# Junshuai-Song/Graph-Embedding

Hardware: AMD Instinct MI355X
Metric: walk-steps/sec (node2vec) (higher is better)
Workload: dtype int32 ids / f64 accept tests

## Files before the change

graph-embedding_amd/csrc/gw_n2v_bitset.hip:

```cpp
#include <hip/hip_runtime.h>
#include <hipcub/hipcub.hpp>

#include <algorithm>
#include <cstdlib>
#include <string>
#include <vector>

#include "gw_device_common.h"

namespace {

constexpr int kB = 256;
constexpr int kBlk = 16;
constexpr int kDirBits = 512;
constexpr int kStage = 16;

constexpr int kPDir = 8;

__host__ __device__ __forceinline__ int64_t bs_ndir(int64_t d) { return d > kDirBits ? (d + kDirBits - 1) / kDirBits : 0; }
__host__ __device__ __forceinline__ int64_t bs_round(int64_t w) { return (w + kBlk - 1) / kBlk * kBlk; }
__host__ __device__ __forceinline__ int64_t bs_boff(int64_t d) {
  return (gw_bs_is_inline((uint32_t)d) || bs_ndir(d) <= kPDir) ? 0 : bs_round(bs_ndir(d));
}
__host__ __device__ __forceinline__ int64_t bs_words(int64_t d) {
  return gw_bs_is_inline((uint32_t)d) ? 0 : bs_boff(d) + bs_round((d + 31) / 32);
}

__device__ __forceinline__ bool bs_has_edge(const gw_dev_graph& G, int64_t rb, int64_t re, int32_t key) {
  if (G.eh) return gw_eh_has(G.eh, rb, re, key);
  if (G.bitmap) {
    const uint32_t h = (uint32_t)key * 0x9E3779B1u;
    const uint64_t bit = 16ull * (uint64_t)rb + (((uint64_t)h * (uint64_t)(16 * (re - rb))) >> 32);
    if (!((G.bitmap[bit >> 5] >> (bit & 31)) & 1u)) return false;
  }
  return gw_row_find(G.nbrs, rb, re, key) >= 0;
}

__host__ __device__ __forceinline__ uint32_t bs_filt_buckets(int64_t ndir, uint32_t d) {
  return 32u * (gw_bs_pw(d) - ((ndir > 0 && ndir <= kPDir) ? 5u : 1u));
}
__host__ __device__ __forceinline__ uint32_t bs_filt_word(int64_t ndir) { return (ndir > 0 && ndir <= kPDir) ? 5u : 1u; }

__device__ __forceinline__ int word_select(uint32_t x, uint32_t j) {
  int pos = 0;
#pragma unroll
  for (int w = 16; w >= 1; w >>= 1) {
    const uint32_t lowc = (uint32_t)__popc(x & ((1u << w) - 1u));
    if (j >= lowc) {
      j -= lowc;
      x >>= w;
      pos += w;
    }
  }
  return pos;
}


enum { BS_LIST = 0, BS_INLINE = 1, BS_EF = 2, BS_REGION = 3 };
constexpr uint32_t kFiltL = 320;

__device__ __forceinline__ int64_t bs_div32(int64_t k, uint32_t d, double inv, bool* exact) {
  int64_t q = (int64_t)((double)k * inv);
  int64_t r = (k << 32) - q * (int64_t)d;
  if (r < 0) {
    --q;
    r += d;
  } else if (r >= (int64_t)d) {
    ++q;
    r -= d;
  }
  *exact = r == 0;
  return q;
}
__device__ __forceinline__ void bs_draw_range(int64_t k, uint32_t d, double inv, uint32_t* ylo, uint32_t* yhi) {
  bool ex;
  *ylo = (uint32_t)bs_div32(k, d, inv, &ex);
  const int64_t q1 = bs_div32(k + 1, d, inv, &ex);
  *yhi = (uint32_t)(q1 - (ex ? 1 : 0));
}
__device__ __forceinline__ double bs_inv32(uint32_t d) { return 4294967296.0 / (double)d; }

__device__ __forceinline__ void bs_filter_only(uint32_t* w, int64_t k, uint32_t d, double inv) {
  uint32_t ulo, uhi;
  bs_draw_range(k, d, inv, &ulo, &uhi);
  const uint32_t b0 = gw_bounded(ulo, kFiltL), b1 = gw_bounded(uhi, kFiltL);
  for (uint32_t b = b0; b <= b1; ++b) atomicOr(&w[b >> 5], 1u << (b & 31));
}
__device__ __forceinline__ int bs_mode(uint32_t c, uint32_t d) {
  return gw_bs_is_list(c, d) ? BS_LIST : gw_bs_is_inline(d) ? BS_INLINE : gw_bs_is_ef(c, d) ? BS_EF : BS_REGION;
}

constexpr uint32_t kDualC = 6;
constexpr uint32_t kMetaDual = 0x40000000u;
constexpr uint32_t kMetaStash = 0x80000000u;

__device__ __forceinline__ uint32_t bs_meta(uint32_t c, uint32_t d) {
  const uint32_t mode = (uint32_t)bs_mode(c, d);
  uint32_t l = 0, U = 0;
  if (mode == BS_EF) {
    l = (uint32_t)gw_bs_ef_l(c, d);
    U = c + ((d - 1) >> l) + 1;
  }
  const uint32_t bblk = (mode == BS_REGION) ? (uint32_t)(bs_boff(d) / kBlk) : 0u;
  return mode | (l << 2) | (U << 7) | (bblk << 16);
}
__device__ __forceinline__ bool bs_dual(uint32_t c, uint32_t c_rev, uint32_t d, uint32_t du) {
  return c <= kDualC && c_rev <= kDualC && d < GW_BS_PACK_D && du < GW_BS_PACK_D;
}
__device__ __forceinline__ uint32_t bs_meta_slot(uint32_t c, uint32_t c_rev, uint32_t d, uint32_t du) {
  return bs_dual(c, c_rev, d, du) ? (kMetaDual | (c_rev << 2)) : bs_meta(c, d);
}

struct BsEmit {
  int mode;
  bool nobits;
  uint32_t* w;
  uint32_t* dir;
  uint16_t* pdir;
  uint32_t* bits;
  int64_t ndir;
  uint32_t d;
  double inv;
  int l;
  uint32_t U;
  __device__ void operator()(int64_t k, uint32_t idx, int64_t kprev) const {
    const uint32_t bit = 1u << (k & 31);
    if (mode == BS_LIST) {
      reinterpret_cast<uint16_t*>(w)[idx] = (uint16_t)k;
    } else if (mode == BS_INLINE) {
      atomicOr(&w[k >> 5], bit);
    } else if (mode == BS_EF) {
      const uint32_t hp = (uint32_t)(k >> l) + idx;
      atomicOr(&w[hp >> 5], 1u << (hp & 31));
      if (l > 0) {
        const uint32_t lowv = (uint32_t)k & ((1u << l) - 1u), off = U + idx * (uint32_t)l, sh = off & 31;
        atomicOr(&w[off >> 5], lowv << sh);
        if (sh + (uint32_t)l > 32u) atomicOr(&w[(off >> 5) + 1], lowv >> (32 - sh));
      }
    } else {
      if (!nobits) atomicOr(&bits[k >> 5], bit);
      set_dir((kprev < 0 ? -1 : kprev / kDirBits) + 1, k / kDirBits, idx);
      uint32_t ulo, uhi;
      bs_draw_range(k, d, inv, &ulo, &uhi);
      const uint32_t F = bs_filt_buckets(ndir, d), w0 = bs_filt_word(ndir);
      const uint32_t b0 = gw_bounded(ulo, F), b1 = gw_bounded(uhi, F);
      for (uint32_t b = b0; b <= b1; ++b) atomicOr(&w[w0 + (b >> 5)], 1u << (b & 31));
    }
  }
  __device__ void set_dir(int64_t g0, int64_t g1, uint32_t count) const {
    if (ndir == 0) return;
    for (int64_t g = g0; g <= g1 && g < ndir; ++g) {
      if (pdir)
        pdir[g] = (uint16_t)count;
      else
        dir[g] = count;
    }
  }
};

__device__ __forceinline__ uint32_t* bs_payload(gw_bs_nbr* en, uint32_t d) { return en->r + (d < GW_BS_PACK_D ? 1 : 2); }
__device__ __forceinline__ uint32_t bs_c(const gw_bs_nbr* en, uint32_t d) { return d < GW_BS_PACK_D ? en->r[0] >> 16 : en->r[1]; }

__device__ __forceinline__ BsEmit bs_emit(gw_bs_nbr* en, uint32_t* reg, const uint64_t* roff, int64_t e, uint32_t c,
                                          uint32_t d) {
  BsEmit E;
  E.mode = bs_mode(c, d);
  E.nobits = false;
  E.w = bs_payload(en, d);
  E.ndir = 0;
  E.dir = E.bits = nullptr;
  E.pdir = nullptr;
  E.d = d;
  E.inv = bs_inv32(d);
  E.l = 0;
  E.U = 0;
  if (E.mode == BS_EF) {
    E.l = gw_bs_ef_l(c, d);
    E.U = c + ((d - 1) >> E.l) + 1;
  } else if (E.mode == BS_REGION) {
    E.ndir = bs_ndir(d);
    E.dir = reg + roff[e];
    E.bits = E.dir + bs_boff(d);
    if (E.ndir <= kPDir) {
      E.pdir = reinterpret_cast<uint16_t*>(E.w + 1);
      E.dir = nullptr;
    }
  }
  return E;
}

__global__ void k_bs_sizes(gw_dev_graph G, const gw_bs_nbr* __restrict__ bsn, uint64_t* __restrict__ sz,
                           int lists_only) {
  const int64_t e = (int64_t)blockIdx.x * blockDim.x + threadIdx.x;
  if (e >= G.nnz) return;
  const uint32_t d = (uint32_t)G.deg[G.nbrs[e]];
  sz[e] = (!lists_only && !gw_bs_is_inline(d) && bs_mode(bs_c(bsn + e, d), d) == BS_REGION)
              ? (uint64_t)bs_words(d) : 0ull;
}

constexpr int kTB = 512;
constexpr int kTW = kTB / 64;
constexpr int kTriH = 4096;
constexpr int kTriS = 2 * kTriH;
constexpr int kTriEB = 512;
constexpr int kTriAhead = 4;
constexpr int32_t kTriNotOwned = INT32_MIN;

constexpr double kBuildProbeRate = 7.7e10;
constexpr double kBuildSlotSeconds = 5.0e-11;

struct TriItem {
  int32_t u, j0;
};

__global__ void k_bs_iota(int64_t n, int32_t* __restrict__ a) {
  const int64_t i = (int64_t)blockIdx.x * blockDim.x + threadIdx.x;
  if (i < n) a[i] = (int32_t)i;
}

__global__ void k_bs_nitems(gw_dev_graph G, const int32_t* __restrict__ order, uint32_t* __restrict__ nit) {
  const int64_t i = (int64_t)blockIdx.x * blockDim.x + threadIdx.x;
  if (i > G.n) return;
  nit[i] = i < G.n ? (uint32_t)((G.deg[order[i]] + kTriEB - 1) / kTriEB) : 0u;
}

__global__ void k_bs_items(gw_dev_graph G, const int32_t* __restrict__ order, const uint32_t* __restrict__ itoff,
                           TriItem* __restrict__ items) {
  const int64_t i = (int64_t)blockIdx.x * blockDim.x + threadIdx.x;
  if (i >= G.n) return;
  const int32_t u = order[i];
  const uint32_t b = itoff[i], e = itoff[i + 1];
  for (uint32_t t = b; t < e; ++t) items[t] = TriItem{u, (int32_t)((t - b) * kTriEB)};
}

struct TriSlot {
  BsEmit E;
  uint32_t* gw;
  bool filt;
  bool dual;
  __device__ void operator()(int64_t k, uint32_t idx, int64_t kprev) const {
    if (filt)
      bs_filter_only(E.w, k, E.d, E.inv);
    else
      E(k, idx, kprev);
  }
};

__device__ __forceinline__ TriSlot tri_slot(gw_bs_nbr* en, uint32_t* reg, const uint64_t* roff, int64_t e, uint32_t c,
                                            uint32_t d, int lists_only, uint32_t* stage, int lane) {
  TriSlot T;
  T.filt = lists_only && bs_mode(c, d) == BS_REGION;
  T.dual = (en->meta & kMetaDual) != 0u;
  T.E = bs_emit(en, reg, roff, e, c, d);
  T.gw = T.E.w;
  T.E.w = stage;
  if (T.E.pdir) T.E.pdir = reinterpret_cast<uint16_t*>(stage + 1);
  if (lane < 12) stage[lane] = 0u;
  __builtin_amdgcn_wave_barrier();
  return T;
}

__device__ __forceinline__ void tri_prologue(const TriSlot& T, int64_t e, const uint64_t* roff, int lane) {
  if (!T.filt && T.E.mode == BS_REGION && lane == 0) T.E.w[0] = (uint32_t)(roff[e] / kBlk);
}

__device__ __forceinline__ void tri_epilogue(const TriSlot& T, int64_t klast, uint32_t c, uint32_t c_rev, int lane) {
  if (T.filt) return;
  if (T.dual) {
    if (lane < 2 * (int)kDualC && (lane < (int)kDualC ? lane >= (int)c : lane - (int)kDualC >= (int)c_rev))
      reinterpret_cast<uint16_t*>(T.E.w)[lane] = 0xFFFFu;
    return;
  }
  if (T.E.mode == BS_LIST && lane >= (int)c && lane < 2 * (int)gw_bs_pw(T.E.d))
    reinterpret_cast<uint16_t*>(T.E.w)[lane] = 0xFFFFu;
  if (T.E.mode != BS_REGION) return;
  for (int64_t g = (klast < 0 ? -1 : klast / kDirBits) + 1 + lane; g < T.E.ndir; g += 64) T.E.set_dir(g, g, c);
}

__device__ __forceinline__ void tri_flush(const TriSlot& T, bool merge, int lane) {
  __builtin_amdgcn_wave_barrier();
  const int pw = (int)gw_bs_pw(T.E.d);
  if (lane < pw) {
    const uint32_t v = T.E.w[lane];
    if (!merge)
      T.gw[lane] = v;
    else if (v)
      atomicOr(&T.gw[lane], v);
  }
  __builtin_amdgcn_wave_barrier();
}

__device__ __forceinline__ void tri_header(gw_bs_nbr* en, uint32_t x, uint32_t d, uint32_t off, uint32_t meta,
                                           uint32_t kp, uint32_t c) {
  *reinterpret_cast<uint4*>(en) = make_uint4(x, d, off, meta);
  *reinterpret_cast<uint2*>(&en->r[0]) =
      d < GW_BS_PACK_D ? make_uint2((kp & 0xFFFFu) | (c << 16), 0u) : make_uint2(kp, c);
}

template <class F>
__device__ __forceinline__ void tri_emit(const F& f, bool on, int64_t pos, uint32_t* cnt, int64_t* last, int lane,
                                         uint16_t* rev, bool need_prev) {
  const unsigned long long m = __ballot(on);
  if (!m) return;
  const unsigned long long lt = m & ((1ull << lane) - 1ull);
  const int32_t p32 = (int32_t)pos;
  int64_t prev = *last;
  if (need_prev) {
    const int32_t pin = __shfl(p32, lt ? 63 - __clzll(lt) : 0, 64);
    if (lt) prev = pin;
  }
  if (on) {
    const uint32_t idx = *cnt + (uint32_t)__popcll(lt);
    f(pos, idx, prev);
    if (rev) rev[kDualC + idx] = (uint16_t)pos;
  }
  *last = __builtin_amdgcn_readlane(p32, 63 - __clzll(m));
  *cnt += (uint32_t)__popcll(m);
}

template <bool FILL>
__global__ void __launch_bounds__(kTB) __attribute__((amdgpu_waves_per_eu(4))) k_bs_tri(gw_dev_graph G, const TriItem* __restrict__ items, uint32_t nitems,
                                                gw_bs_nbr* __restrict__ bsn,
                                                const uint64_t* __restrict__ roff, uint32_t* __restrict__ reg,
                                                int lists_only) {
  __shared__ int32_t s_key[kTriS];
  __shared__ uint16_t s_pos[kTriS];
  __shared__ uint32_t s_cuv[kTriEB], s_cvu[kTriEB], s_cur[kTriEB];
  __shared__ int32_t s_luv[kTriEB], s_lvu[kTriEB], s_kp[kTriEB];
  __shared__ int32_t s_nx[kTriEB];
  __shared__ uint32_t s_stage[kTW][2][12];
  __shared__ uint32_t s_win[kTW][kTriH / 32];
  const int tid = threadIdx.x, lane = tid & 63, wave = tid >> 6;
  const int diag = kGwDiag ? (lists_only >> 8) : 0;
  lists_only &= 1;
  if (FILL) {
    for (int i = lane; i < kTriH / 32; i += 64) s_win[wave][i] = 0u;
  }
  for (uint32_t item = blockIdx.x; item < nitems; item += gridDim.x) {
    if (item != blockIdx.x) __syncthreads();
    const TriItem it = items[item];
    const int32_t u = it.u;
    const int64_t ub = G.offsets[u], du = G.offsets[u + 1] - ub;
    const int64_t j0 = it.j0, j1 = min(du, j0 + (int64_t)kTriEB);
    const int nch = (int)((du + kTriH - 1) / kTriH);
    const int64_t hk = min(du, (int64_t)kTriH);
    int lg = 6;
    while ((1 << lg) < 2 * hk) ++lg;
    const uint32_t S = 1u << lg, smask = S - 1u;
    const int sh = 32 - lg;
    for (int ch = 0; ch < nch; ++ch) {
      const int64_t p0 = (int64_t)ch * kTriH, p1 = min(du, p0 + kTriH);
      if (ch > 0) __syncthreads();
      for (uint32_t i = tid; i < S; i += kTB) s_key[i] = -1;
      __syncthreads();
      for (int64_t i = tid; i < p1 - p0; i += kTB) {
        const int32_t x = G.nbrs[ub + p0 + i];
        uint32_t h = ((uint32_t)x * 0x9E3779B1u) >> sh;
        while (atomicCAS(&s_key[h], -1, x) != -1) h = (h + 1) & smask;
        s_pos[h] = (uint16_t)i;
      }
      __syncthreads();
      const int32_t hi = ch == nch - 1 ? INT32_MAX : G.nbrs[ub + p1 - 1];
      int64_t jp = j0 + wave;
      int32_t pv_n = jp + kTW < j1 ? G.nbrs[ub + jp + kTW] : 0;
      int32_t pv = 0;
      int64_t pvb = 0, pve = 0;
      if (jp < j1) {
        pv = G.nbrs[ub + jp];
        pvb = G.offsets[pv];
        pve = G.offsets[pv + 1];
      }
      for (int64_t j = jp; j < j1; j += kTW) {
        const int32_t v = pv;
        const int64_t vb = pvb, dv = pve - pvb;
        if (j + kTW < j1) {
          pv = pv_n;
          pvb = G.offsets[pv];
          pve = G.offsets[pv + 1];
        }
        if (j + 2 * kTW < j1) pv_n = G.nbrs[ub + j + 2 * kTW];
        const int li = (int)(j - j0);
        if (ch > 0) {
          const int32_t nx = s_nx[li];
          if (nx == kTriNotOwned || (ch + 1 < nch && nx > hi)) continue;
        }
        if (!(du > dv || (du == dv && u <= v))) {
          if (nch > 1 && lane == 0) s_nx[li] = kTriNotOwned;
          continue;
        }
        const int64_t e = ub + j;
        uint32_t cuv = 0, cvu = 0, cur = 0;
        int64_t luv = -1, lvu = -1, kp = -1;
        if (ch > 0) {
          cuv = s_cuv[li];
          cvu = s_cvu[li];
          cur = s_cur[li];
          luv = s_luv[li];
          lvu = s_lvu[li];
          kp = s_kp[li];
        }
        int64_t k = (int64_t)cur + lane;
        int32_t x = k < dv ? G.nbrs[vb + k] : INT32_MAX;
        int32_t xa[kTriAhead - 1];
#pragma unroll
        for (int r = 0; r < kTriAhead - 1; ++r) xa[r] = k + 64 * (r + 1) < dv ? G.nbrs[vb + k + 64 * (r + 1)] : INT32_MAX;
        TriSlot Tuv, Tvu;
        int64_t er = -1;
        bool vu_win = false;
        if (FILL) {
          gw_bs_nbr* en = bsn + e;
          const uint32_t c = bs_c(en, (uint32_t)dv);
          Tuv = tri_slot(en, reg, roff, e, c, (uint32_t)dv, lists_only, s_stage[wave][0], lane);
          Tuv.E.nobits = true;
          if (ch == 0) tri_prologue(Tuv, e, roff, lane);
          if (u != v) {
            const uint32_t kpv = (uint32_t)dv < GW_BS_PACK_D ? (en->r[0] & 0xFFFFu) : en->r[0];
            er = vb + kpv;
            gw_bs_nbr* enr = bsn + er;
            const uint32_t cr = bs_c(enr, (uint32_t)du);
            Tvu = tri_slot(enr, reg, roff, er, cr, (uint32_t)du, lists_only, s_stage[wave][1], lane);
            if (ch == 0) tri_prologue(Tvu, er, roff, lane);
            vu_win = !Tvu.filt && Tvu.E.mode == BS_REGION;
            Tvu.E.nobits = vu_win;
          }
        }
        int32_t nx = INT32_MAX;
        for (;;) {
          const int64_t kf = k + 64 * kTriAhead;
          const int32_t xf = kf < dv ? G.nbrs[vb + kf] : INT32_MAX;
          const bool inr = k < dv && x <= hi;
          bool hit = false;
          uint32_t pu = 0;
          if (inr) {
            uint32_t h = ((uint32_t)x * 0x9E3779B1u) >> sh;
            for (;;) {
              const int32_t kk = s_key[h];
              if (kk == x) {
                hit = true;
                pu = (uint32_t)p0 + s_pos[h];
                break;
              }
              if (kk == -1) break;
              h = (h + 1) & smask;
            }
          }
          const unsigned long long mu = __ballot(inr && x == u);
          if (mu) kp = (int64_t)cur + (__ffsll(mu) - 1);
          const bool cu = hit && x != u;
          const bool cv = hit && x != v && u != v;
          if (FILL && !(diag & 1)) {
            if (!(diag & 2) && !Tuv.filt && Tuv.E.mode == BS_REGION) {
              const unsigned long long m = __ballot(cu);
              if (m) {
                const uint32_t sh = cur & 31u;
                const unsigned long long lo = m << sh;
                const uint32_t hi3 = sh ? (uint32_t)(m >> (64 - sh)) : 0u;
                const uint32_t wv = lane == 0 ? (uint32_t)lo : lane == 1 ? (uint32_t)(lo >> 32) : hi3;
                if (lane < 3 && wv) atomicOr(&Tuv.E.bits[(cur >> 5) + lane], wv);
              }
            }
            const bool dual = u != v && Tuv.dual;
            tri_emit(Tuv, cu, k, &cuv, &luv, lane, dual ? reinterpret_cast<uint16_t*>(Tvu.E.w) : nullptr,
                     !Tuv.filt && Tuv.E.mode == BS_REGION);
            if (u != v) {
              tri_emit(Tvu, cv, (int64_t)pu, &cvu, &lvu, lane, dual ? reinterpret_cast<uint16_t*>(Tuv.E.w) : nullptr,
                       !Tvu.filt && Tvu.E.mode == BS_REGION);
              if (cv && vu_win && !(diag & 2)) atomicOr(&s_win[wave][(pu - (uint32_t)p0) >> 5], 1u << (pu & 31u));
            }
          } else if (!FILL) {
            const unsigned long long m1 = __ballot(cu), m2 = __ballot(cv);
            cuv += (uint32_t)__popcll(m1);
            cvu += (uint32_t)__popcll(m2);
          }
          const int nin = __popcll(__ballot(inr));
          cur += (uint32_t)nin;
          if (nin < 64) {
            nx = __shfl(x, nin, 64);
            break;
          }
          k += 64;
          x = xa[0];
#pragma unroll
          for (int r = 0; r < kTriAhead - 2; ++r) xa[r] = xa[r + 1];
          xa[kTriAhead - 2] = xf;
        }
        if (FILL && ch + 1 == nch) {
          tri_epilogue(Tuv, luv, cuv, cvu, lane);
          if (u != v) tri_epilogue(Tvu, lvu, cvu, cuv, lane);
        }
        if (FILL && !(diag & 4)) {
          tri_flush(Tuv, nch > 1, lane);
          if (u != v) tri_flush(Tvu, nch > 1, lane);
          if (vu_win) {
            __builtin_amdgcn_wave_barrier();
            for (int i = lane; i < kTriH / 32; i += 64) {
              const uint32_t wv = s_win[wave][i];
              if (wv) {
                Tvu.E.bits[(p0 >> 5) + i] = wv;
                s_win[wave][i] = 0u;
              }
            }
            __builtin_amdgcn_wave_barrier();
          }
        }
        if (ch + 1 < nch) {
          if (lane == 0) {
            s_cuv[li] = cuv;
            s_cvu[li] = cvu;
            s_cur[li] = cur;
            s_luv[li] = (int32_t)luv;
            s_lvu[li] = (int32_t)lvu;
            s_kp[li] = (int32_t)kp;
            s_nx[li] = nx;
          }
          continue;
        }
        if (!FILL) {
          const uint32_t k32 = kp >= 0 ? (uint32_t)kp : 0xFFFFFFFFu;
          if (lane == 0)
            tri_header(bsn + e, (uint32_t)v, (uint32_t)dv, (uint32_t)vb,
                       bs_meta_slot(cuv, u != v ? cvu : 0xFFFFu, (uint32_t)dv, (uint32_t)du), k32, cuv);
          if (lane == 1 && u != v && kp >= 0)
            tri_header(bsn + vb + kp, (uint32_t)u, (uint32_t)du, (uint32_t)ub,
                       bs_meta_slot(cvu, cuv, (uint32_t)du, (uint32_t)dv), (uint32_t)j, cvu);
        }
      }
    }
  }
}

template <int NW>
__device__ __forceinline__ int regs_select(const uint32_t* wd, uint32_t j) {
  uint32_t S = 0, T = 0, below = 0, x = wd[0];
#pragma unroll
  for (int t = 0; t < NW; ++t) {
    S += (uint32_t)__popc(wd[t]);
    const bool le = S <= j;
    T += le ? 1u : 0u;
    below = le ? S : below;
    if (t + 1 < NW) x = le ? wd[t + 1] : x;
  }
  return 32 * (int)T + word_select(x, j - below);
}

constexpr int kPW = 11;
__device__ __forceinline__ uint32_t pickw(const uint32_t (&pl)[kPW], uint32_t idx) {
  const bool b0 = idx & 1u, b1 = idx & 2u, b2 = idx & 4u, b3 = idx & 8u;
  const uint32_t a0 = b0 ? pl[1] : pl[0], a1 = b0 ? pl[3] : pl[2], a2 = b0 ? pl[5] : pl[4];
  const uint32_t a3 = b0 ? pl[7] : pl[6], a4 = b0 ? pl[9] : pl[8];
  const uint32_t c0 = b1 ? a1 : a0, c1 = b1 ? a3 : a2, c2 = b1 ? pl[10] : a4;
  const uint32_t e0 = b2 ? c1 : c0;
  return b3 ? c2 : e0;
}

__device__ __forceinline__ uint32_t bits32(const uint32_t (&pl)[kPW], uint32_t pos) {
  const uint32_t w = pos >> 5;
  return __builtin_amdgcn_alignbit(pickw(pl, w + 1), pickw(pl, w), pos & 31u);
}

__device__ __forceinline__ bool ef_bucket_has(const uint32_t (&pl)[kPW], uint32_t U, uint32_t l, uint32_t s,
                                              uint32_t e0, uint32_t k, uint32_t lw) {
  uint32_t hw = bits32(pl, s), run = 0;
  while (hw == 0xFFFFFFFFu && run < 320u) {
    run += 32u;
    hw = bits32(pl, s + run);
  }
  run += (uint32_t)__builtin_ctz(~hw);
  if (l == 0) return run > 0;
  const uint32_t mask = (1u << l) - 1u, lowk = k & mask;
  uint32_t o = 0;
  for (uint32_t i = 0; i < run; ++i) {
    if (o + l > 32u) {
      lw = bits32(pl, U + (e0 + i) * l);
      o = 0;
    }
    const uint32_t f = (lw >> o) & mask;
    if (f >= lowk) return f == lowk;
    o += l;
  }
  return false;
}

__device__ __forceinline__ bool list_has(const uint32_t (&pl)[kPW], uint32_t k, bool dual = false) {
  bool hit = false;
#pragma unroll
  for (int t = 0; t < kPW; ++t)
    hit |= (t < (int)kDualC / 2 || !dual) && ((pl[t] & 0xFFFFu) == k || (pl[t] >> 16) == k);
  return hit;
}

struct BsParams {
  double a_p, a_q;
  uint32_t k0, k1, pk0, pk1;
  uint32_t diag;
};

__device__ __forceinline__ void unpack_entry(const uint32_t (&E)[16], uint32_t* kp, uint32_t* c, uint32_t (&pl)[kPW]) {
  const bool packed = E[1] < GW_BS_PACK_D;
  *kp = packed ? (E[4] & 0xFFFFu) : E[4];
  *c = packed ? (E[4] >> 16) : E[5];
#pragma unroll
  for (int q = 0; q < kPW - 1; ++q) pl[q] = packed ? E[5 + q] : E[6 + q];
  pl[kPW - 1] = packed ? E[15] : 0u;
}

__device__ __forceinline__ uint4 coop_piece(uint64_t sec, int lane, int j) {
  const int src = 16 * j + (lane >> 2);
  const uint64_t sj = ((uint64_t)(uint32_t)__shfl((int)(uint32_t)(sec >> 32), src, 64) << 32) |
                      (uint32_t)__shfl((int)(uint32_t)sec, src, 64);
  uint4 r = make_uint4(0u, 0u, 0u, 0u);
  if (sj != 0ull) r = reinterpret_cast<const uint4*>(sj)[lane & 3];
  return r;
}

__global__ void __launch_bounds__(kB) __attribute__((amdgpu_waves_per_eu(5, 5)))
k_walk_bitset(gw_dev_graph G, BsParams P, int L, int64_t walk_begin, int64_t walk_count, int shuffle,
              int32_t* __restrict__ out, int32_t* __restrict__ lens, unsigned long long* __restrict__ counters) {
  __shared__ int32_t s_stage[kB / 64][kStage][64];
  __shared__ uint4 s_ex[kB / 64][64];
  const int lane = threadIdx.x & 63;
  const int wv = threadIdx.x >> 6;
  int32_t* stage = &s_stage[wv][0][lane];
  uint4* ex = s_ex[wv];
  const uint4* __restrict__ ents = reinterpret_cast<const uint4*>(G.bs_nbr);

  const int64_t i = (int64_t)blockIdx.x * blockDim.x + threadIdx.x;
  const bool valid = i < walk_count;
  unsigned long long my_steps = 0;
  uint32_t my_trials = 0;
  const int64_t w = walk_begin + (valid ? i : 0);
  int32_t cur = -1;
  int len = L;
  if (valid) {
    const uint64_t it = (uint64_t)w / (uint64_t)G.n;
    const uint64_t pos = (uint64_t)w % (uint64_t)G.n;
    const uint64_t sp = shuffle ? gw_feistel_perm(pos, (uint64_t)G.n, P.pk0, P.pk1, (uint32_t)it) : pos;
    cur = G.order[sp];
    len = 1;
  }
  const bool vec_ok = (L & 3) == 0;
  const uint32_t c0 = (uint32_t)w, c1 = (uint32_t)((uint64_t)w >> 32);
  stage[0] = cur;
  uint32_t trial = 0;
  uint32_t b = 0, d = 0;
  if (valid) {
    b = (uint32_t)G.offsets[cur];
    d = (uint32_t)(G.offsets[cur + 1] - G.offsets[cur]);
  }
  uint32_t c = 0, kp = 0, meta = 0;
  uint32_t pl[kPW];
#pragma unroll
  for (int t = 0; t < kPW; ++t) pl[t] = 0xFFFFFFFFu;
  uint32_t ph = 0, t = 0;
  int64_t g = 0;
  uint32_t dw0 = 0u, dw1 = 0u, kb = 0u;
  uint32_t dg_iter = 0, dg_act = 0;
  for (;;) {
    const bool active = len < L && d != 0;
    if (__ballot(active) == 0ull) break;
    if (kGwDiag && (P.diag & 64)) {
      ++dg_iter;
      dg_act += active ? 1u : 0u;
    }
    uint32_t slot = 0xFFFFFFFFu;
    bool spec = false;
    uint32_t sw = 0u, sbit = 0u;
    uint64_t sec = 0ull;
    bool isblk = false;
    bool virt = false;
    if (active) {
      const uint32_t mode = meta & 3u;
      const int efl = (int)((meta >> 2) & 31u);
      const uint32_t efU = (meta >> 7) & 511u;
      const uint32_t* hreg = G.bs_region + (uint64_t)pl[0] * kBlk;
      const int64_t ndir = bs_ndir(d);
      int64_t k = 0;
      bool acc = false;
      if (ph == 3) {
        k = kb;
        acc = true;
        ph = 0;
      } else if (ph == 1) {
        const uint32_t lo = dw0, hi = g + 1 < ndir ? dw1 : c;
        if (t < lo || t >= hi) {
          g += t < lo ? -1 : 1;
          dw0 = hreg[g];
          dw1 = g + 1 < ndir ? hreg[g + 1] : 0u;
        } else {
          t -= lo;
          ph = 2;
        }
      } else {
        const gw_u4 u = gw_philox(c0, c1, (uint32_t)len, trial, P.k0, P.k1);
        ++trial;
        int op = 0;
        uint32_t j = 0;
        if (len == 1) {
          k = (int64_t)gw_index(u.x, u.z, d);
          acc = true;
        } else {
          bool other = trial > 1;
          if (!other) {
            const double Z = (P.a_p + (double)c) + (double)((int64_t)d - 1 - (int64_t)c) * P.a_q;
            const double r = gw_u01(u.x) * Z;
            if (r < P.a_p) {
              k = kp;
              acc = true;
            } else if (r - P.a_p < (double)c) {
              j = (uint32_t)(r - P.a_p);
              if (j >= c) j = c - 1;
              op = 1;
            } else {
              other = true;
            }
          }
          if (other) {
            k = (int64_t)gw_index(u.y, u.z, d);
            op = 2;
          }
        }
        if (kGwDiag && P.diag) {
          if (op == 1 && (P.diag & 1)) {
            k = (int64_t)((uint64_t)j * (uint64_t)d / c);
            acc = true;
            op = 0;
          }
          if (op == 2 && (P.diag & 2)) {
            acc = k != (int64_t)kp;
            op = 0;
          }
        }
        bool common = false;
        const uint32_t eh = (uint32_t)k >> efl;
        const bool ef_mem = op == 2 && mode == BS_EF && eh <= efU - c;
        int pos = 0;
        if ((op == 1 && (mode == BS_INLINE || mode == BS_EF)) || (ef_mem && eh > 0)) {
          const bool inv = op == 2;
          uint32_t wp[kPW];
#pragma unroll
          for (int q = 0; q < kPW; ++q) wp[q] = inv ? ~pl[q] : pl[q];
          pos = regs_select<kPW>(wp, inv ? eh - 1 : j);
        }
        const uint32_t es = (ef_mem && eh > 0) ? (uint32_t)pos + 1u : 0u;
        const uint32_t fb = gw_bounded(u.y, bs_filt_buckets(ndir, d));
        const uint32_t wpos = mode == BS_LIST     ? 16u * j
                              : mode == BS_INLINE ? (uint32_t)k
                              : mode == BS_EF     ? efU + (op == 1 ? j : es - eh) * (uint32_t)efl
                                                  : 32u * bs_filt_word(ndir) + fb;
        const uint32_t win = bits32(pl, wpos);
        if (op == 1) {
          if (mode == BS_INLINE) {
            k = (int64_t)pos;
            acc = true;
          } else if (mode == BS_EF) {
            k = ((int64_t)(uint32_t)(pos - (int)j) << efl) | (win & ((1u << efl) - 1u));
            acc = true;
          } else if (mode == BS_LIST) {
            k = (int64_t)(win & 0xFFFFu);
            acc = true;
          } else {
            if (ndir > kPDir) {
              g = (int64_t)((float)j * (float)ndir * __builtin_amdgcn_rcpf((float)c));
              if (g >= ndir) g = ndir - 1;
              dw0 = hreg[g];
              dw1 = g + 1 < ndir ? hreg[g + 1] : 0u;
              t = j;
              ph = 1;
            } else {
              uint32_t lo = 0;
              g = 0;
#pragma unroll
              for (int q = 1; q < kPDir; ++q) {
                const uint32_t dq = (pl[1 + (q >> 1)] >> (16 * (q & 1))) & 0xFFFFu;
                const bool in = q < ndir && dq <= j;
                g += in ? 1 : 0;
                lo = in ? dq : lo;
              }
              t = j - lo;
              ph = 2;
            }
          }
        } else if (op == 2) {
          if (mode == BS_LIST) {
            common = c != 0u && list_has(pl, (uint32_t)k, (meta & kMetaDual) != 0u);
          } else if (mode == BS_INLINE) {
            common = win & 1u;
          } else if (mode == BS_EF) {
            common = ef_mem && ef_bucket_has(pl, efU, (uint32_t)efl, es, es - eh, (uint32_t)k, win);
          } else if (k != (int64_t)kp && trial < (1u << 24)) {
            if (win & 1u) {
              sw = (kGwDiag && (P.diag & 8)) ? G.bs_region[((uint32_t)k >> 5) & 0xFFFFu]
                                : hreg[(meta >> 16) * kBlk + (k >> 5)];
              sbit = (uint32_t)(k & 31);
              spec = true;
            }
          }
          acc = (k != (int64_t)kp && !common) || trial >= (1u << 24);
        }
      }
      if (ph == 2 && !acc) {
        sec = (kGwDiag && (P.diag & 4)) ? (uint64_t)(G.bs_region + kBlk * ((pl[0] + (uint32_t)g) & 0xFFFu))
                           : (uint64_t)(hreg + ((meta >> 16) + (uint32_t)g) * kBlk);
        isblk = true;
      }
      if (acc) {
        if ((meta & kMetaStash) && k == (int64_t)kp) {
          virt = true;
        } else {
          slot = b + (uint32_t)k;
          sec = (uint64_t)(ents + (uint64_t)slot * 4u);
        }
      }
    }
    const uint4 r0 = coop_piece(sec, lane, 0), r1 = coop_piece(sec, lane, 1);
    const uint4 r2 = coop_piece(sec, lane, 2), r3 = coop_piece(sec, lane, 3);
    if (spec && ((sw >> sbit) & 1u)) {
      slot = 0xFFFFFFFFu;
      sec = 0ull;
    }
    uint32_t E[16];
#pragma unroll
    for (int q = 0; q < 4; ++q) {
      __builtin_amdgcn_wave_barrier();
      if ((lane & 3) == q) {
        ex[lane >> 2] = r0;
        ex[16 + (lane >> 2)] = r1;
        ex[32 + (lane >> 2)] = r2;
// ... 121 lines not shown

__device__ __forceinline__ bool payload_has(const uint32_t (&pl)[kPW], uint32_t meta, uint32_t c, uint32_t k) {
  const uint32_t mode = meta & 3u;
  const uint32_t efl = (meta >> 2) & 31u, efU = (meta >> 7) & 511u;
  if (mode == BS_LIST) return list_has(pl, k, (meta & 0x8000u) != 0u);
  const uint32_t eh = k >> efl;
  uint32_t es = 0;
  if (mode == BS_EF && eh > 0) {
    uint32_t wp[kPW];
#pragma unroll
    for (int q = 0; q < kPW; ++q) wp[q] = ~pl[q];
    es = (uint32_t)regs_select<kPW>(wp, eh - 1) + 1u;
  }
  const uint32_t win = bits32(pl, mode == BS_INLINE ? k : efU + (es - eh) * efl);
  if (mode == BS_INLINE) return win & 1u;
  return eh <= efU - c && ef_bucket_has(pl, efU, efl, es, es - eh, k, win);
}

__global__ void __launch_bounds__(kB) __attribute__((amdgpu_waves_per_eu(5, 5)))
k_walk_listed(gw_dev_graph G, LsParams P, int L, int64_t walk_begin, int64_t walk_count, int shuffle,
              int32_t* __restrict__ out, int32_t* __restrict__ lens, unsigned long long* __restrict__ counters) {
  __shared__ int32_t s_stage[kB / 64][kStage][64];
  __shared__ uint4 s_ex[kB / 64][64];
  const int lane = threadIdx.x & 63;
  const int wv = threadIdx.x >> 6;
  int32_t* stage = &s_stage[wv][0][lane];
  uint4* ex = s_ex[wv];
  const uint4* __restrict__ ents = reinterpret_cast<const uint4*>(G.bs_nbr);

  const int64_t i = (int64_t)blockIdx.x * blockDim.x + threadIdx.x;
  const bool valid = i < walk_count;
  unsigned long long my_steps = 0, my_trials = 0;
  const int64_t w = walk_begin + (valid ? i : 0);
  int32_t cur = -1, prev = -1;
  int len = L;
  if (valid) {
    const uint64_t it = (uint64_t)w / (uint64_t)G.n;
    const uint64_t pos = (uint64_t)w % (uint64_t)G.n;
    const uint64_t sp = shuffle ? gw_feistel_perm(pos, (uint64_t)G.n, P.pk0, P.pk1, (uint32_t)it) : pos;
    cur = G.order[sp];
    len = 1;
  }
  const bool vec_ok = (L & 3) == 0;
  const uint32_t c0 = (uint32_t)w, c1 = (uint32_t)((uint64_t)w >> 32);
  stage[0] = cur;
  uint32_t trial = 0;
  uint32_t b = 0, d = 0, pb = 0, pd = 0;
  if (valid) {
    b = (uint32_t)G.offsets[cur];
    d = (uint32_t)(G.offsets[cur + 1] - G.offsets[cur]);
  }
  uint32_t meta = BS_REGION;
  uint32_t pl[kPW];
#pragma unroll
  for (int t = 0; t < kPW; ++t) pl[t] = 0u;
  bool pend = false;
  int32_t px = 0;
  uint32_t pdx = 0, poff = 0, pmeta = 0;
  double t = 0.0;
  bool filt = false;
  uint32_t fb = 0;
  for (;;) {
    const bool active = len < L && d != 0;
    if (__ballot(active) == 0ull) break;
    uint64_t sec = 0ull;
    uint32_t k = 0;
    bool ret = false;
    uint32_t hs = 0;
    int4 h0 = make_int4(-1, -1, -1, -1);
    if (pend) {
      hs = gw_eh_slot(px, pd);
      h0 = gw_eh_row(G.eh, pb)[hs];
    }
    if (active && !pend) {
      if (len == 1) {
        const gw_u4 u = gw_philox(c0, c1, 1u, 0u, P.k0, P.k1);
        trial = 1;
        k = gw_index(u.x, u.z, d);
      } else {
        const gw_u4 u = gw_philox(c0, c1, (uint32_t)len, trial, P.k0, P.k1);
        ++trial;
        const double A = P.M * (double)d + P.extra;
        if (P.extra > 0.0 && gw_u01(u.z) * A < P.extra) {
          ret = true;
        } else {
          k = gw_index(u.x, u.y, d);
          t = gw_u01(u.w) * P.M;
          fb = (uint32_t)(((uint64_t)u.x * kFiltL) >> 32);
        }
      }
      if (!ret) sec = (uint64_t)(ents + (uint64_t)(b + k) * 4u);
    }
    const uint4 r0 = coop_piece(sec, lane, 0), r1 = coop_piece(sec, lane, 1);
    const uint4 r2 = coop_piece(sec, lane, 2), r3 = coop_piece(sec, lane, 3);
    uint32_t E[16];
#pragma unroll
    for (int q = 0; q < 4; ++q) {
      __builtin_amdgcn_wave_barrier();
      if ((lane & 3) == q) {
        ex[lane >> 2] = r0;
        ex[16 + (lane >> 2)] = r1;
        ex[32 + (lane >> 2)] = r2;
        ex[48 + (lane >> 2)] = r3;
      }
      __builtin_amdgcn_wave_barrier();
      const uint4 v = ex[lane];
      E[4 * q] = v.x;
      E[4 * q + 1] = v.y;
      E[4 * q + 2] = v.z;
      E[4 * q + 3] = v.w;
    }
    __builtin_amdgcn_wave_barrier();
    bool acc = ret, take = false;
    if (pend) {
      const int r0 = gw_eh_scan(h0, px);
      const bool adj = r0 > 0 || (r0 < 0 && gw_eh_has_from(G.eh, pb, pd, hs, px));
      acc = t < (adj ? 1.0 : P.a_q) || trial >= (1u << 24);
      pend = false;
    } else if (sec != 0ull) {
      const int32_t next = (int32_t)E[0];
      if (len == 1) {
        acc = true;
      } else if (next == prev) {
        acc = t < P.h_prev;
      } else if (t < P.lo) {
        acc = true;
      } else if ((meta & 3u) != BS_REGION) {
        acc = t < (payload_has(pl, meta, meta >> 16, k) ? 1.0 : P.a_q);
      } else if (filt && !((pickw(pl, fb >> 5) >> (fb & 31)) & 1u)) {
        acc = t < P.a_q;
      } else if (G.eh) {
        pend = true;
        filt = false;
        px = next;
      } else {
        acc = t < (bs_has_edge(G, pb, (int64_t)pb + pd, next) ? 1.0 : P.a_q);
      }
      if (trial >= (1u << 24) && !pend) acc = true;
      take = true;
    }
    if (take && (pend || acc)) {
      uint32_t ekp, ec;
      unpack_entry(E, &ekp, &ec, pl);
      pdx = E[1];
      poff = E[2];
      pmeta = (E[3] & 0x7FFFu) | ((E[3] & kMetaDual) ? 0x8000u : 0u) | (min(ec, 0xFFFFu) << 16);
    }
    bool ready = false;
    int flen = 0;
    if (acc) {
      my_trials += trial;
      trial = 0;
      const int32_t next = ret ? prev : take ? (int32_t)E[0] : px;
      const uint32_t ob = pb, od = pd;
      prev = cur;
      pb = b;
      pd = d;
      cur = next;
      if (ret) {
        b = ob;
        d = od;
        meta = BS_REGION;
      } else {
        d = pdx;
        b = poff;
        meta = pmeta;
      }
      filt = !ret && (meta & 3u) == BS_REGION;
      stage[64 * (len & (kStage - 1))] = cur;
      ready = (len & (kStage - 1)) == kStage - 1;
      flen = len;
      ++len;
    }
    const unsigned long long rm = __ballot(ready);
    if (rm) {
      if (vec_ok) {
        const int nready = __popcll(rm);
        int32_t* ids = reinterpret_cast<int32_t*>(ex);
        __builtin_amdgcn_wave_barrier();
        if (ready)
          ids[__builtin_amdgcn_mbcnt_hi((uint32_t)(rm >> 32), __builtin_amdgcn_mbcnt_lo((uint32_t)rm, 0u))] = lane;
        __builtin_amdgcn_wave_barrier();
        const int32_t* sw = &s_stage[wv][0][0];
        for (int j = 0; 16 * j < nready; ++j) {
          const int q = 16 * j + (lane >> 2), p4 = 4 * (lane & 3);
          const int r = ids[q < nready ? q : nready - 1];
          const int lr = __shfl(flen, r, 64);
          const int64_t ir = ((int64_t)__shfl((int)(i >> 32), r, 64) << 32) | (uint32_t)__shfl((int)i, r, 64);
          if (q < nready) {
            const int4 v = make_int4(sw[64 * p4 + r], sw[64 * (p4 + 1) + r], sw[64 * (p4 + 2) + r], sw[64 * (p4 + 3) + r]);
            *reinterpret_cast<int4*>(out + ir * (int64_t)L + (lr - (kStage - 1)) + p4) = v;
          }
        }
        __builtin_amdgcn_wave_barrier();
      } else if (ready) {
        int32_t* dst = out + i * (int64_t)L + (flen - (kStage - 1));
        for (int j = 0; j < kStage; ++j) dst[j] = stage[64 * j];
      }
    }
  }
  if (valid) {
    int32_t* row = out + i * (int64_t)L;
    const int base = len & ~(kStage - 1);
    for (int t = base; t < len; ++t) row[t] = stage[64 * (t - base)];
    for (int t = len; t < L; ++t) row[t] = -1;
    if (lens) lens[i] = len;
    my_steps = (unsigned long long)(len - 1);
  }
  if (counters) {
    for (int off = 32; off > 0; off >>= 1) {
      my_steps += __shfl_down(my_steps, off, 64);
      my_trials += __shfl_down(my_trials, off, 64);
    }
    if ((threadIdx.x & 63) == 0) {
      atomicAdd(&counters[0], my_steps);
      atomicAdd(&counters[1], my_trials);
    }
  }
}

template <typename T>
int bs_alloc(gw_graph* g, T** p, int64_t count) {
  *p = nullptr;
  if (count <= 0) count = 1;
  hipError_t e = hipMalloc((void**)p, sizeof(T) * (size_t)count);
  if (e != hipSuccess) {
    g->err = std::string("hipMalloc(bitset ") + std::to_string(sizeof(T) * (size_t)count) + " B): " + hipGetErrorString(e);
    *p = nullptr;
    return GW_ERR_NOMEM;
  }
  return GW_OK;
}

template <typename T>
void bs_free(T*& p) {
  if (p) (void)hipFree(p);
  p = nullptr;
}

}

void gw_dev_bitset_release(gw_graph* g) {
  bs_free(g->d.bs_region);
  bs_free(g->d.bs_nbr);
}

__device__ __forceinline__ int64_t bs_row_of(const gw_dev_graph& G, int64_t e) {
  int64_t lo = 0, hi = G.n;
  while (lo < hi) {
    const int64_t mid = (lo + hi) >> 1;
    if (G.offsets[mid + 1] <= e)
      lo = mid + 1;
    else
      hi = mid;
  }
  return lo;
}

constexpr int kWorkChunk = 16;
__global__ void k_bs_work(gw_dev_graph G, unsigned long long* __restrict__ acc) {
  const int64_t e0 = ((int64_t)blockIdx.x * blockDim.x + threadIdx.x) * kWorkChunk;
  unsigned long long w = 0;
  if (e0 < G.nnz) {
    const int64_t e1 = e0 + kWorkChunk < G.nnz ? e0 + kWorkChunk : G.nnz;
    int64_t u = bs_row_of(G, e0);
    int64_t ue = G.offsets[u + 1];
    int64_t du = ue - G.offsets[u];
    for (int64_t e = e0; e < e1; ++e) {
      if (e >= ue) {
        u = bs_row_of(G, e);
        ue = G.offsets[u + 1];
        du = ue - G.offsets[u];
      }
      const int32_t v = G.nbrs[e];
      const int64_t dv = G.deg[v];
      if (du > dv || (du == dv && u <= v)) w += (unsigned long long)dv;
    }
  }
  for (int o = 32; o > 0; o >>= 1) w += __shfl_down(w, o, 64);
  if ((threadIdx.x & 63) == 0 && w) atomicAdd(acc, w);
}

int gw_dev_bitset_build(gw_graph* g, int64_t budget_bytes, bool lists_only) {
  gw_dev_graph& d = g->d;
  gw_dev_bitset_release(g);
  const int64_t nnz = g->nnz, n = g->n;
  if (nnz == 0) return GW_OK;
  if (nnz >= (int64_t)0xFFFFFFFF) {
    g->err = "bitset mode supports < 2^32 - 1 adjacency entries: use GW_N2V_REJECTION";
    return GW_ERR_CAPACITY;
  }
  if (nnz * (int64_t)sizeof(gw_bs_nbr) > budget_bytes) {
    g->err = "bitset entries need " + std::to_string(nnz * (int64_t)sizeof(gw_bs_nbr)) + " B; over the " +
             std::to_string(budget_bytes) + " B budget: use GW_N2V_REJECTION";
    return GW_ERR_CAPACITY;
  }
  if (g->max_degree >= ((int64_t)1 << 27)) {
    g->err = "bitset mode supports vertex degrees < 2^27: use GW_N2V_REJECTION";
    return GW_ERR_UNSUPPORTED;
  }
  int rc;
  uint64_t* sz = nullptr;
  uint64_t* roff = nullptr;
  int32_t *ids = nullptr, *order = nullptr;
  int32_t* dkey = nullptr;
  uint32_t* nit = nullptr;
  uint32_t* itoff = nullptr;
  TriItem* items = nullptr;
  void* tmp = nullptr;
  auto cleanup = [&]() {
    bs_free(sz);
    bs_free(roff);
    bs_free(ids);
    bs_free(order);
    bs_free(nit);
    bs_free(itoff);
    bs_free(items);
    bs_free(tmp);
    bs_free(dkey);
  };
  auto fail = [&](int code) {
    cleanup();
    gw_dev_bitset_release(g);
    return code;
  };
#define BS_TRY(expr)                                                 \
  do {                                                               \
    hipError_t _e = (expr);                                          \
    if (_e != hipSuccess) {                                          \
      g->err = std::string(#expr) + ": " + hipGetErrorString(_e);    \
      return fail(GW_ERR_DEVICE);                                    \
    }                                                                \
  } while (0)
  if ((rc = bs_alloc(g, &d.bs_nbr, nnz)) || (rc = bs_alloc(g, &ids, n)) ||
      (rc = bs_alloc(g, &order, n)) || (rc = bs_alloc(g, &nit, n + 1)) || (rc = bs_alloc(g, &itoff, n + 1)))
    return fail(rc);
  const unsigned gn = (unsigned)((n + kB - 1) / kB), gn1 = (unsigned)((n + 1 + kB - 1) / kB);
  BS_TRY(hipMemset(d.bs_nbr, 0, (size_t)nnz * sizeof(gw_bs_nbr)));
  k_bs_iota<<<gn, kB>>>(n, ids);
  BS_TRY(hipGetLastError());
  size_t tb = 0, tb2 = 0;
  BS_TRY(hipcub::DeviceRadixSort::SortPairsDescending(nullptr, tb, (const int32_t*)nullptr, (int32_t*)nullptr,
                                                      (const int32_t*)nullptr, (int32_t*)nullptr, (int)n));
  BS_TRY(hipcub::DeviceScan::ExclusiveSum(nullptr, tb2, nit, itoff, (int)(n + 1)));
  if ((rc = bs_alloc(g, (char**)&tmp, (int64_t)std::max(tb, tb2) + 1))) return fail(rc);
  if ((rc = bs_alloc(g, &dkey, n))) return fail(rc);
  BS_TRY(hipcub::DeviceRadixSort::SortPairsDescending(tmp, tb, d.deg, dkey, ids, order, (int)n));
  int bs_diag = 0;
  if (const char* dg = GW_DIAG_ENV("GW_DIAG_BS_FILL")) bs_diag = std::atoi(dg);
  int64_t nbig = 0;
  if (bs_diag & 8) {
    std::vector<int32_t> hk((size_t)n);
    BS_TRY(hipMemcpy(hk.data(), dkey, (size_t)n * 4, hipMemcpyDeviceToHost));
    while (nbig < n && hk[(size_t)nbig] > 64) ++nbig;
  }
  bs_free(dkey);
  k_bs_nitems<<<gn1, kB>>>(d, order, nit);
  BS_TRY(hipGetLastError());
  BS_TRY(hipcub::DeviceScan::ExclusiveSum(tmp, tb2, nit, itoff, (int)(n + 1)));
  uint32_t nitems = 0, isplit = 0;
  BS_TRY(hipMemcpy(&nitems, itoff + n, sizeof(uint32_t), hipMemcpyDeviceToHost));
  if (bs_diag & 8) BS_TRY(hipMemcpy(&isplit, itoff + nbig, sizeof(uint32_t), hipMemcpyDeviceToHost));
  if ((rc = bs_alloc(g, &items, std::max<int64_t>(nitems, 1)))) return fail(rc);
  k_bs_items<<<gn, kB>>>(d, order, itoff, items);
  BS_TRY(hipGetLastError());
  bs_free(tmp);
  bs_free(ids);
  bs_free(order);
  bs_free(nit);
  bs_free(itoff);
  auto tri = [&](bool fill, const TriItem* it, uint32_t cnt) {
    if (!cnt) return;
    const unsigned tgrid = std::min<uint32_t>(cnt, 1u << 20);
    if (fill)
      k_bs_tri<true><<<tgrid, kTB>>>(d, it, cnt, d.bs_nbr, roff, d.bs_region, (lists_only ? 1 : 0) | (bs_diag << 8));
    else
      k_bs_tri<false><<<tgrid, kTB>>>(d, it, cnt, d.bs_nbr, nullptr, nullptr, lists_only ? 1 : 0);
  };
  auto tri_all = [&](bool fill) {
    if (bs_diag & 8) {
      tri(fill, items, isplit);
      tri(fill, items + isplit, nitems - isplit);
    } else {
      tri(fill, items, nitems);
    }
  };
  tri_all(false);
  BS_TRY(hipGetLastError());
  if ((rc = bs_alloc(g, &sz, nnz + 1)) || (rc = bs_alloc(g, &roff, nnz + 1))) return fail(rc);
  const unsigned grid = (unsigned)((nnz + kB - 1) / kB);
  k_bs_sizes<<<grid, kB>>>(d, d.bs_nbr, sz, lists_only ? 1 : 0);
  BS_TRY(hipGetLastError());
  BS_TRY(hipMemset(sz + nnz, 0, sizeof(uint64_t)));
  size_t tmpb = 0;
  BS_TRY(hipcub::DeviceScan::ExclusiveSum(nullptr, tmpb, sz, roff, nnz + 1));
  if ((rc = bs_alloc(g, (char**)&tmp, (int64_t)tmpb + 1))) return fail(rc);
  BS_TRY(hipcub::DeviceScan::ExclusiveSum(tmp, tmpb, sz, roff, nnz + 1));
  BS_TRY(hipDeviceSynchronize());
  bs_free(tmp);
  bs_free(sz);
  uint64_t words = 0;
  BS_TRY(hipMemcpy(&words, roff + nnz, sizeof(uint64_t), hipMemcpyDeviceToHost));
  const int64_t need = (int64_t)words * 4 + nnz * (int64_t)sizeof(gw_bs_nbr);
  if (need > budget_bytes) {
    g->err = "per-edge bitsets need " + std::to_string(need) + " B; over the " + std::to_string(budget_bytes) +
             " B budget: use GW_N2V_REJECTION";
    return fail(GW_ERR_CAPACITY);
  }
  if (words == 0) words = 1;
  if ((rc = bs_alloc(g, &d.bs_region, (int64_t)words))) return fail(rc);
  BS_TRY(hipMemset(d.bs_region, 0, (size_t)words * 4));
  tri_all(true);
  BS_TRY(hipGetLastError());
  BS_TRY(hipDeviceSynchronize());
#undef BS_TRY
  cleanup();
  g->bitset_words = (int64_t)words;
  return GW_OK;
}

double gw_bitset_build_model_s(gw_graph* g) {
  if (g->bs_model_s >= 0.0) return g->bs_model_s;
  unsigned long long* acc = nullptr;
  if (hipMalloc((void**)&acc, sizeof(unsigned long long)) != hipSuccess) return -1.0;
  unsigned long long w = 0;
  bool ok = hipMemset(acc, 0, sizeof w) == hipSuccess;
  if (ok && g->nnz > 0) {
    const int64_t threads = (g->nnz + kWorkChunk - 1) / kWorkChunk;
    k_bs_work<<<(unsigned)((threads + kB - 1) / kB), kB>>>(g->d, acc);
    ok = hipGetLastError() == hipSuccess;
  }
  ok = ok && hipMemcpy(&w, acc, sizeof w, hipMemcpyDeviceToHost) == hipSuccess;
  (void)hipFree(acc);
  if (!ok) return -1.0;
  g->bs_model_s = 2.0 * (double)w / kBuildProbeRate + (double)g->nnz * kBuildSlotSeconds;
  return g->bs_model_s;
}

int gw_dev_walk_bitset_launch(gw_graph* g, int L, uint64_t seed, int64_t walk_begin, int64_t walk_count,
                              int shuffle, int32_t* out_dev, int32_t* len_dev, uint64_t* counters_dev,
                              void* stream) {
  BsParams P;
  P.a_p = 1.0 / g->p;
  P.a_q = 1.0 / g->q;
  P.k0 = (uint32_t)seed;
  P.k1 = (uint32_t)(seed >> 32) ^ GW_TAG_N2V_STEP;
  P.pk0 = (uint32_t)seed;
  P.pk1 = (uint32_t)(seed >> 32) ^ GW_TAG_N2V_PERM;
  const char* dg = GW_DIAG_ENV("GW_DIAG_BS");
  P.diag = dg ? (uint32_t)atoi(dg) : 0u;
  if (const char* ns = GW_DIAG_ENV("GW_DIAG_NO_STORE")) P.diag |= ns[0] == '1' ? 32u : 0u;
  const unsigned grid = (unsigned)std::max<int64_t>(1, (walk_count + kB - 1) / kB);
  k_walk_bitset<<<grid, kB, 0, (hipStream_t)stream>>>(g->d, P, L, walk_begin, walk_count, shuffle, out_dev,
                                                       len_dev, (unsigned long long*)counters_dev);
  GW_HIP_TRY(hipGetLastError());
  return GW_OK;
}

int gw_dev_walk_listed_launch(gw_graph* g, int L, uint64_t seed, int64_t walk_begin, int64_t walk_count,
                              int shuffle, int32_t* out_dev, int32_t* len_dev, uint64_t* counters_dev,
                              void* stream) {
  LsParams P;
  const double a_p = 1.0 / g->p;
  P.a_q = 1.0 / g->q;
  P.M = std::max(1.0, P.a_q);
  P.lo = std::min(1.0, P.a_q);
  P.extra = a_p > P.M ? a_p - P.M : 0.0;
  P.h_prev = std::min(a_p, P.M);
  P.k0 = (uint32_t)seed;
  P.k1 = (uint32_t)(seed >> 32) ^ GW_TAG_N2V_STEP;
  P.pk0 = (uint32_t)seed;
  P.pk1 = (uint32_t)(seed >> 32) ^ GW_TAG_N2V_PERM;
  const unsigned grid = (unsigned)std::max<int64_t>(1, (walk_count + kB - 1) / kB);
  k_walk_listed<<<grid, kB, 0, (hipStream_t)stream>>>(g->d, P, L, walk_begin, walk_count, shuffle, out_dev,
                                                       len_dev, (unsigned long long*)counters_dev);
  GW_HIP_TRY(hipGetLastError());
  return GW_OK;
}
```

Before: 34.71 billion.

## Precompute per-edge build records to avoid scattered reads in bitset fill pass

The first triangle pass now writes a 32-byte per-edge record holding both directions' counts, the reverse position and, after a new gather kernel, both region offsets. The fill pass then reads this record with two vector loads in place of chasing bsn headers and roff for the edge and its reverse. k_bs_sizes also reads the degree from the bsn entry, avoiding a double indirection. This trades an extra nnz*32 B buffer and one extra kernel for fewer dependent scattered loads. It only affects bitset build time, which may or may not count toward walk-steps/sec.

```diff
diff --git a/graph-embedding_amd/csrc/gw_n2v_bitset.hip b/graph-embedding_amd/csrc/gw_n2v_bitset.hip
--- a/graph-embedding_amd/csrc/gw_n2v_bitset.hip
+++ b/graph-embedding_amd/csrc/gw_n2v_bitset.hip
@@ -161,8 +161,7 @@
 __device__ __forceinline__ uint32_t* bs_payload(gw_bs_nbr* en, uint32_t d) { return en->r + (d < GW_BS_PACK_D ? 1 : 2); }
 __device__ __forceinline__ uint32_t bs_c(const gw_bs_nbr* en, uint32_t d) { return d < GW_BS_PACK_D ? en->r[0] >> 16 : en->r[1]; }
 
-__device__ __forceinline__ BsEmit bs_emit(gw_bs_nbr* en, uint32_t* reg, const uint64_t* roff, int64_t e, uint32_t c,
-                                          uint32_t d) {
+__device__ __forceinline__ BsEmit bs_emit(gw_bs_nbr* en, uint32_t* reg, uint64_t ro, uint32_t c, uint32_t d) {
   BsEmit E;
   E.mode = bs_mode(c, d);
   E.nobits = false;
@@ -179,7 +178,7 @@
     E.U = c + ((d - 1) >> E.l) + 1;
   } else if (E.mode == BS_REGION) {
     E.ndir = bs_ndir(d);
-    E.dir = reg + roff[e];
+    E.dir = reg + ro;
     E.bits = E.dir + bs_boff(d);
     if (E.ndir <= kPDir) {
       E.pdir = reinterpret_cast<uint16_t*>(E.w + 1);
@@ -193,7 +192,7 @@
                            int lists_only) {
   const int64_t e = (int64_t)blockIdx.x * blockDim.x + threadIdx.x;
   if (e >= G.nnz) return;
-  const uint32_t d = (uint32_t)G.deg[G.nbrs[e]];
+  const uint32_t d = bsn[e].d;
   sz[e] = (!lists_only && !gw_bs_is_inline(d) && bs_mode(bs_c(bsn + e, d), d) == BS_REGION)
               ? (uint64_t)bs_words(d) : 0ull;
 }
@@ -213,6 +212,13 @@
   int32_t u, j0;
 };
 
+struct alignas(32) TriRec {
+  uint32_t c_uv, c_vu;
+  uint32_t kp_uv, pad;
+  uint64_t roff_uv, roff_vu;
+};
+static_assert(sizeof(TriRec) == 32, "build record: two 16 B halves");
+
 __global__ void k_bs_iota(int64_t n, int32_t* __restrict__ a) {
   const int64_t i = (int64_t)blockIdx.x * blockDim.x + threadIdx.x;
   if (i < n) a[i] = (int32_t)i;
@@ -231,6 +237,24 @@
   const int32_t u = order[i];
   const uint32_t b = itoff[i], e = itoff[i + 1];
   for (uint32_t t = b; t < e; ++t) items[t] = TriItem{u, (int32_t)((t - b) * kTriEB)};
+}
+
+__global__ void __launch_bounds__(kTriEB) k_bs_rec_roff(gw_dev_graph G, const TriItem* __restrict__ items,
+                                                        uint32_t nitems, const uint64_t* __restrict__ roff,
+                                                        TriRec* __restrict__ rec) {
+  for (uint32_t item = blockIdx.x; item < nitems; item += gridDim.x) {
+    const TriItem it = items[item];
+    const int32_t u = it.u;
+    const int64_t ub = G.offsets[u], du = G.offsets[u + 1] - ub;
+    const int64_t j = (int64_t)it.j0 + threadIdx.x;
+    if (j >= du) continue;
+    const int32_t v = G.nbrs[ub + j];
+    const int64_t vb = G.offsets[v], dv = G.offsets[v + 1] - vb;
+    if (!(du > dv || (du == dv && u <= v))) continue;
+    const int64_t e = ub + j;
+    const uint64_t ro_vu = u != v ? roff[vb + rec[e].kp_uv] : 0ull;
+    *reinterpret_cast<ulonglong2*>(&rec[e].roff_uv) = make_ulonglong2(roff[e], ro_vu);
+  }
 }
 
 struct TriSlot {
@@ -246,12 +270,12 @@
   }
 };
 
-__device__ __forceinline__ TriSlot tri_slot(gw_bs_nbr* en, uint32_t* reg, const uint64_t* roff, int64_t e, uint32_t c,
-                                            uint32_t d, int lists_only, uint32_t* stage, int lane) {
+__device__ __forceinline__ TriSlot tri_slot(gw_bs_nbr* en, uint32_t* reg, uint64_t ro, uint32_t c, uint32_t d, bool dual,
+                                            int lists_only, uint32_t* stage, int lane) {
   TriSlot T;
   T.filt = lists_only && bs_mode(c, d) == BS_REGION;
-  T.dual = (en->meta & kMetaDual) != 0u;
-  T.E = bs_emit(en, reg, roff, e, c, d);
+  T.dual = dual;
+  T.E = bs_emit(en, reg, ro, c, d);
   T.gw = T.E.w;
   T.E.w = stage;
   if (T.E.pdir) T.E.pdir = reinterpret_cast<uint16_t*>(stage + 1);
@@ -260,8 +284,8 @@
   return T;
 }
 
-__device__ __forceinline__ void tri_prologue(const TriSlot& T, int64_t e, const uint64_t* roff, int lane) {
-  if (!T.filt && T.E.mode == BS_REGION && lane == 0) T.E.w[0] = (uint32_t)(roff[e] / kBlk);
+__device__ __forceinline__ void tri_prologue(const TriSlot& T, uint64_t ro, int lane) {
+  if (!T.filt && T.E.mode == BS_REGION && lane == 0) T.E.w[0] = (uint32_t)(ro / kBlk);
 }
 
 __device__ __forceinline__ void tri_epilogue(const TriSlot& T, int64_t klast, uint32_t c, uint32_t c_rev, int lane) {
@@ -321,7 +345,7 @@
 template <bool FILL>
 __global__ void __launch_bounds__(kTB) __attribute__((amdgpu_waves_per_eu(4))) k_bs_tri(gw_dev_graph G, const TriItem* __restrict__ items, uint32_t nitems,
                                                 gw_bs_nbr* __restrict__ bsn,
-                                                const uint64_t* __restrict__ roff, uint32_t* __restrict__ reg,
+                                                TriRec* __restrict__ rec, uint32_t* __restrict__ reg,
                                                 int lists_only) {
   __shared__ int32_t s_key[kTriS];
   __shared__ uint16_t s_pos[kTriS];
@@ -405,21 +429,19 @@
 #pragma unroll
         for (int r = 0; r < kTriAhead - 1; ++r) xa[r] = k + 64 * (r + 1) < dv ? G.nbrs[vb + k + 64 * (r + 1)] : INT32_MAX;
         TriSlot Tuv, Tvu;
-        int64_t er = -1;
         bool vu_win = false;
         if (FILL) {
-          gw_bs_nbr* en = bsn + e;
-          const uint32_t c = bs_c(en, (uint32_t)dv);
-          Tuv = tri_slot(en, reg, roff, e, c, (uint32_t)dv, lists_only, s_stage[wave][0], lane);
+          const uint4 rh = *reinterpret_cast<const uint4*>(rec + e);
+          const ulonglong2 ro = *reinterpret_cast<const ulonglong2*>(&rec[e].roff_uv);
+          const uint64_t ro_uv = ro.x, ro_vu = ro.y;
+          const bool dual = u != v && bs_dual(rh.x, rh.y, (uint32_t)dv, (uint32_t)du);
+          Tuv = tri_slot(bsn + e, reg, ro_uv, rh.x, (uint32_t)dv, dual, lists_only, s_stage[wave][0], lane);
           Tuv.E.nobits = true;
-          if (ch == 0) tri_prologue(Tuv, e, roff, lane);
+          if (ch == 0) tri_prologue(Tuv, ro_uv, lane);
           if (u != v) {
-            const uint32_t kpv = (uint32_t)dv < GW_BS_PACK_D ? (en->r[0] & 0xFFFFu) : en->r[0];
-            er = vb + kpv;
-            gw_bs_nbr* enr = bsn + er;
-            const uint32_t cr = bs_c(enr, (uint32_t)du);
-            Tvu = tri_slot(enr, reg, roff, er, cr, (uint32_t)du, lists_only, s_stage[wave][1], lane);
-            if (ch == 0) tri_prologue(Tvu, er, roff, lane);
+            const int64_t er = vb + rh.z;
+            Tvu = tri_slot(bsn + er, reg, ro_vu, rh.y, (uint32_t)du, dual, lists_only, s_stage[wave][1], lane);
+            if (ch == 0) tri_prologue(Tvu, ro_vu, lane);
             vu_win = !Tvu.filt && Tvu.E.mode == BS_REGION;
             Tvu.E.nobits = vu_win;
           }
@@ -523,6 +545,7 @@
           if (lane == 1 && u != v && kp >= 0)
             tri_header(bsn + vb + kp, (uint32_t)u, (uint32_t)du, (uint32_t)ub,
                        bs_meta_slot(cvu, cuv, (uint32_t)du, (uint32_t)dv), (uint32_t)j, cvu);
+          if (lane == 2) *reinterpret_cast<uint4*>(rec + e) = make_uint4(cuv, cvu, k32, 0u);
         }
       }
     }
@@ -1250,6 +1273,7 @@
   int rc;
   uint64_t* sz = nullptr;
   uint64_t* roff = nullptr;
+  TriRec* rec = nullptr;
   int32_t *ids = nullptr, *order = nullptr;
   int32_t* dkey = nullptr;
   uint32_t* nit = nullptr;
@@ -1259,6 +1283,7 @@
   auto cleanup = [&]() {
     bs_free(sz);
     bs_free(roff);
+    bs_free(rec);
     bs_free(ids);
     bs_free(order);
     bs_free(nit);
@@ -1317,13 +1342,14 @@
   bs_free(order);
   bs_free(nit);
   bs_free(itoff);
+  if ((rc = bs_alloc(g, &rec, nnz))) return fail(rc);
   auto tri = [&](bool fill, const TriItem* it, uint32_t cnt) {
     if (!cnt) return;
     const unsigned tgrid = std::min<uint32_t>(cnt, 1u << 20);
     if (fill)
-      k_bs_tri<true><<<tgrid, kTB>>>(d, it, cnt, d.bs_nbr, roff, d.bs_region, (lists_only ? 1 : 0) | (bs_diag << 8));
+      k_bs_tri<true><<<tgrid, kTB>>>(d, it, cnt, d.bs_nbr, rec, d.bs_region, (lists_only ? 1 : 0) | (bs_diag << 8));
     else
-      k_bs_tri<false><<<tgrid, kTB>>>(d, it, cnt, d.bs_nbr, nullptr, nullptr, lists_only ? 1 : 0);
+      k_bs_tri<false><<<tgrid, kTB>>>(d, it, cnt, d.bs_nbr, rec, nullptr, lists_only ? 1 : 0);
   };
   auto tri_all = [&](bool fill) {
     if (bs_diag & 8) {
@@ -1355,6 +1381,9 @@
              " B budget: use GW_N2V_REJECTION";
     return fail(GW_ERR_CAPACITY);
   }
+  if (nitems) k_bs_rec_roff<<<std::min<uint32_t>(nitems, 1u << 20), kTriEB>>>(d, items, nitems, roff, rec);
+  BS_TRY(hipGetLastError());
+  bs_free(roff);
   if (words == 0) words = 1;
   if ((rc = bs_alloc(g, &d.bs_region, (int64_t)words))) return fail(rc);
   BS_TRY(hipMemset(d.bs_region, 0, (size_t)words * 4));
```

Measured after the change: 34.60 billion. About the same (-0.3%).
